# deno750/TSP_Optimization

Measured on AMD Instinct MI355X. Metric: 2opt_edge_pair_evals_per_sec, higher is better.
Workload: dtype f64

## Files before the change

tsp_optimization_amd/csrc/tsp_internal.hpp:

```cpp
#pragma once
#include <hip/hip_runtime.h>
#include <time.h>

#include <cstdint>
#include <cstdio>
#include <cstdlib>
#include <cstring>
#include <type_traits>
#include <vector>

#include "../../include/tsp_hip.h"
#include "tsp_dist.hpp"
#include "exh_arith.hpp"
#include "exh_decide.hpp"

namespace tsp {

struct alignas(16) Partial {
    double delta;
    int i, j;
};
static_assert(sizeof(Partial) == 16, "Partial must be 16 bytes");

struct alignas(16) TourState {
    int ci, cj;
    int chunk_rows;
    int done;
    double obj;
    double seen_cost;
    long long sweeps, evals, moves, reversed, pairs_scanned, steps;
    int parity, pending, mv_pa, mv_pb;
    long long lane_pairs, tier1_pairs, exact_pairs, staged_recs;
    int hit_rows;
    int open;
    int pad1, pad2;
};

constexpr int kScanThreads = 256;
constexpr int kApplyThreads = 1024;

}

#define TSP_SWITCH_LIST(X)                                                                                                  \
    X(ENGINE) X(CLUSTER_BLOCKS) X(CLUSTER_MIN_ROWS) X(CLUSTER_MAX_ROWS) X(CLUSTER_HIT_CAP) X(CLUSTER_SPIN_LIMIT)            \
    X(CLUSTER_SPIN_MS) X(CLUSTER_COPIES) X(CLUSTER_TILE_ROWS) X(CLUSTER_XCD_LOCAL) X(CLUSTER_ALLOW_OVERSUB) X(CLUSTER_DEBUG) X(CLUSTER_PROBE) X(CLUSTER_FIRST_SORTED) X(TABU_DENSE)     \
    X(LDS_PROBE) X(LDS_MIN_ROWS) X(LDS_EDGE_CACHE) X(NO_ICOORD) X(NO_FILTER) X(NO_PRUNE) X(SORTED_MIN_N)      \
    X(SWEEP_BLOCKS) X(SWEEP_TABLE) X(BEST_ROWS_PER_BLOCK) X(BEST_RECS) X(FIRST_GRID_ROWS) X(FIRST_MIN_ROWS)                \
    X(FIRST_MAX_ROWS) X(CONSTRUCT_GLOBAL) X(CONSTRUCT_NN) X(CLUSTER_FS_ROWS) X(LDS_F32_MIN_N) X(EXH_POS) X(TABU_INKERNEL) X(OROPT_FULL)
namespace tsp {
enum SwitchId {
#define TSP_SW_ENUM(name) SW_##name,
    TSP_SWITCH_LIST(TSP_SW_ENUM)
#undef TSP_SW_ENUM
    SW_COUNT
};
struct Switches {
    int v[SW_COUNT];
    bool has[SW_COUNT];
    int get(SwitchId k, int dflt) const { return has[k] ? v[k] : dflt; }
};
void read_switches(Switches *sw);
}
#define TSP_SW(inst_, NAME, dflt) ((inst_)->sw.get(tsp::SW_##NAME, (dflt)))


struct tsp_dev_ctx {
    int device = 0;
    hipStream_t stream = nullptr;
// ... 80 lines not shown
    bool exh_hot = false;
    int exh_share[4] = {0, 0, 0, 0};
    int exh_gens = 0;
    tsp::ExhDeal *d_exh_deal = nullptr;
    tsp::ExhCand *d_exh_cand = nullptr;
    int exh_lds = 0;
    int exh_blocks = 0;
    int *d_pairtab = nullptr;
    int *d_ticket = nullptr;
    int *d_row_ticket = nullptr;
    tsp::Partial *d_row_slot = nullptr;
    int *d_row_evals = nullptr;
    int max_tile_rows = 0;
    int *d_slot_evals = nullptr;
    unsigned long long *d_cl_slots = nullptr;
    size_t cl_slot_words = 0;
    int cl_C = 0;
    long long *d_cl_stats = nullptr;
    unsigned cl_epoch = 0;
    int *d_cl_pairtab = nullptr;
    int cl_ntests = 0;
    int *d_order_snap = nullptr;
    std::vector<double> h_obj_snap;
    int *d_kick_result = nullptr;
    int *h_kick_result = nullptr;
    int *d_chain = nullptr, *h_chain = nullptr;
    bool h_state_fresh = false;
    int *h_cl_err = nullptr;
    bool tabu_list_run = false;
    int *d_order0 = nullptr;
    std::vector<double> h_obj0;
    std::vector<int> h_order_buf;
    tsp::TourState *h_state = nullptr;
    int first_grid_rows = 32;
    int first_max_rows2 = 2048;
    int first_min_rows = 8;
    int best_rows_per_block = 32;
    int use_recs = 1;
    double device_ms = 0.0;
};

namespace tsp {
void set_last_error(const char *what, hipError_t e, const char *file, int line);
void set_last_error_text(const char *text);

template <typename T>
struct DevBuf {
    T *p = nullptr;
    DevBuf() = default;
    DevBuf(const DevBuf &) = delete;
    DevBuf &operator=(const DevBuf &) = delete;
    ~DevBuf() { if (p) (void)hipFree(p); }
    hipError_t alloc(size_t count) { return hipMalloc(&p, sizeof(T) * count); }
    operator T *() const { return p; }
};
}
namespace tsp {
struct HkTree {
    const int *d_elo = nullptr, *d_ehi = nullptr;
    const double *d_ew = nullptr, *d_pi = nullptr;
    double W = 0.0;
    long long rounds = 0;
    float device_ms = 0.f;
};
struct TabuRide {
    tsp_dev_tabu *tabu = nullptr;
// ... 73 lines not shown
```

tsp_optimization_amd/csrc/two_opt_exh.hpp:

```cpp
#pragma once
#include "two_opt_step.hpp"
#include "exh_arith.hpp"
#include "exh_decide.hpp"

#pragma clang fp contract(off)

namespace tsp {

#ifdef TSP_STAMPS
__device__ unsigned long long g_exh_w[8192 * 4];
__device__ unsigned long long g_exh_t[8];
__device__ unsigned long long g_exh_f[8192];
#endif

constexpr int kExhPad = 1152;
constexpr int kRowBatch = 4;
constexpr int kExhRJ = 4;

template <int WT>
constexpr bool exh_metric() { return WT == WT_EUC_2D_ICOORD || WT == WT_CEIL_2D_ICOORD || WT == WT_ATT_ICOORD; }

template <int WT>
constexpr int exh_mode() { return WT == WT_EUC_2D_ICOORD ? EXH_NINT : (WT == WT_CEIL_2D_ICOORD ? EXH_CEIL : EXH_ATT); }

// ... 89 lines not shown
    __syncthreads();
    d = s_d[0]; key = s_k[0];
    for (int w = 1; w < kScanThreads / 64; ++w)
        if (better(s_d[w], s_k[w], d, key)) { d = s_d[w]; key = s_k[w]; }
    if (key == kNoKey || !(d < 0)) return {0, -1, -1};
    const int delta = (int)d;
    bool ambiguous = false;
    for (int w = 0; w < kScanThreads / 64; ++w)
        ambiguous = ambiguous || (s_k[w] != kNoKey && s_d[w] == d && (s_amb[w] != 0 || s_k[w] != key));
    if (ambiguous) {
        ExhIdBest ib;
#pragma unroll
        for (int k = 0; k < kExhCandPU; ++k) exh_fold_ids(ib, one.c[k], delta, id_at);
        if (two) {
#pragma unroll
            for (int k = 0; k < kExhCandPU; ++k) exh_fold_ids(ib, more.c[k], delta, id_at);
        }
        u64 idkey = ib.idkey;
        double unused = 0.0;
        block_argmin<false>(unused, idkey, s_d, s_k);
        if (ib.idkey == idkey) s_pair = ib.poskey;
        __syncthreads();
        key = s_pair;
    }
    return {1, exh_key_hi(key), exh_key_lo(key)};
}

__device__ __forceinline__ SweepDecision exh_decision(const ExhMove &m) {
    SweepDecision d;
    d.found = 1; d.pa = m.pa; d.pb = m.pb; d.L = m.L;
    return d;
}

template <int WT, bool INT, bool HOT>
__global__ __launch_bounds__(kScanThreads) void k_move_pos(const TourState *__restrict__ states, const ExhCand *__restrict__ cands,
                                                           const ExhRec *__restrict__ rec_old, int cand_per_tour, int n,
                                                           ExhRec *__restrict__ rec, TourState *__restrict__ states_next,
                                                           const double2 *__restrict__ coord, int *orders, int *poss, int *orders2,
                                                           int *poss2) {
    static_assert(exh_metric<WT>() && INT, "integer-coordinate metrics only (integer costs: the tour cost needs no staging)");
    __shared__ double s_d[kScanThreads / 64];
    __shared__ u64 s_k[kScanThreads / 64];
    const int tour = blockIdx.y;
    const TourState *st = states + tour;
    const bool writer = blockIdx.x == 0 && threadIdx.x == 0;
    const ExhCand *cand = cands + (size_t)tour * cand_per_tour;
    const ExhCandLoads first = exh_cand_load(cand, cand_per_tour, threadIdx.x);
    int done = st->done, is_open = st->open, parity = st->parity, pending = st->pending, mv_pa = st->mv_pa, mv_pb = st->mv_pb;
    __builtin_amdgcn_sched_barrier(0);
    const int args_null = (int)(coord == nullptr) | (int)(orders == nullptr) | (int)(poss == nullptr) | (int)(orders2 == nullptr) |
                          (int)(poss2 == nullptr) | (int)(states_next == nullptr) | (int)(rec_old == nullptr) | (int)(rec == nullptr);
    asm volatile("" : "+s"(done), "+s"(is_open), "+s"(parity), "+s"(pending), "+s"(mv_pa), "+s"(mv_pb) : "s"(n), "s"(args_null));
    exh_cand_pin(first);
    if (done) {
        if (writer) states_next[tour] = *st;
        return;
    }
    const size_t base = (size_t)tour * n, pbase = (size_t)tour * (n + kExhPad);
    MoveView mv = move_view(parity, pending, mv_pa, mv_pb, orders + base, poss + base, orders2 + base, poss2 + base, n);
    const ExhRec *__restrict__ old = rec_old + pbase;
    const bool open = is_open != 0;
    SweepDecision dec;
    ExhPair pr = {0, -1, -1};
    if (open) {
        pr = exh_decide(first, cand, cand_per_tour, [&](int p) { if constexpr (HOT) return old[p].id; else return mv.order[p]; }, s_d, s_k);
        if (!pr.found) {
            if (blockIdx.x != 0) return;
            const double cost = tour_cost_block<WT, INT>(coord, mv.order, mv.pos, n, s_d, nullptr);
            if (writer) {
                TourState z = *st;
                sweep_count(z, dec, n, cost);
                z.pending = 0;
                states_next[tour] = z;
            }
            return;
        }
    }
    const int k = blockIdx.x * kScanThreads + threadIdx.x;
    if (k >= n + kExhPad) return;
    int u;
    ExhRec r;
    if constexpr (HOT) {
        ExhMove m1 = {mv_pa, mv_pb, mv.pa1, mv.L}, m2 = m1;
        if (open) { m1 = exh_orient(pr.p, pr.q, n, true); m2 = exh_orient(pr.p, pr.q, n, false); }
        const ExhPerm pm1 = exh_perm(k, n, m1.pa1, m1.L), pm2 = exh_perm(k, n, m2.pa1, m2.L);
        const ExhRec ra1 = old[pm1.a], rb1 = old[pm1.b], ra2 = old[pm2.a], rb2 = old[pm2.b];
        const int wrap = old[n].eprev;
        int idp = 0, idq = 1;
        if (open) { idp = old[pr.p].id; idq = old[pr.q].id; }
        __builtin_amdgcn_sched_barrier(0);
        asm volatile("" : : "v"(ra1.m2x), "v"(ra1.m2y), "v"(ra1.nrm), "v"(ra1.eprev), "v"(rb1.m2x), "v"(rb1.m2y), "v"(rb1.nrm),
                     "v"(rb1.eprev), "v"(rb1.id), "v"(wrap));
        asm volatile("" : : "v"(ra2.m2x), "v"(ra2.m2y), "v"(ra2.nrm), "v"(ra2.eprev), "v"(rb2.m2x), "v"(rb2.m2y), "v"(rb2.nrm),
                     "v"(rb2.eprev), "v"(rb2.id), "v"(idp), "v"(idq));
        const bool p_first = idp < idq;
        const ExhMove m = p_first ? m1 : m2;
        r = exh_perm_rec<exh_mode<WT>()>(p_first ? pm1 : pm2, p_first ? ra1 : ra2, p_first ? rb1 : rb2, wrap,
                                         [](double v) { return __builtin_amdgcn_sqrt(v); });
        u = r.id;
        mv.L = m.L; mv.pa1 = m.pa1;
        if (open) dec = exh_decision(m);
    } else {
        if (open) {
            const ExhMove m = exh_orient(pr.p, pr.q, n, mv.order[pr.p] < mv.order[pr.q]);
            mv.L = m.L; mv.pa1 = m.pa1;
            dec = exh_decision(m);
        }
        u = k < n ? mv.node_at(k) : (k == n ? mv.node_at(0) : -1);
        const int v = k >= 1 && k <= n ? mv.node_at(k - 1) : -1;
        const double2 c0 = coord[0];
        double2 cu = make_double2(c0.x - 6.0e6, c0.y - 6.0e6);
        int len = 0;
        if (u >= 0) cu = coord[u];
        if (v >= 0) { const double2 cv = coord[v]; len = (int)dist_xy<WT, INT>(cv.x, cv.y, cu.x, cu.y); }
        exh_rec_xy(cu.x - c0.x, cu.y - c0.y, r);
        r.eprev = len;
        r.id = u;
    }
    if (mv.L > 0 && k < n) {
        int *o_new = (parity ? orders : orders2) + base, *p_new = (parity ? poss : poss2) + base;
        o_new[k] = u;
        p_new[u] = k;
    }
    rec[pbase + k] = r;
    if (writer) {
        TourState z = *st;
        if (open) sweep_count(z, dec, n, 0.0);
        if (mv.L > 0) z.parity ^= 1;
        z.pending = 0;
        states_next[tour] = z;
    }
}

template <int WT, bool INT>
__global__ __launch_bounds__(kScanThreads) void k_exh_close(const double2 *__restrict__ coord, const int *orders, const int *poss,
                                                            const int *orders2, const int *poss2, TourState *states,
                                                            const ExhCand *__restrict__ cands, int cand_per_tour, int n) {
    static_assert(exh_metric<WT>() && INT, "integer-coordinate metrics only");
    __shared__ double s_d[kScanThreads / 64];
    __shared__ u64 s_k[kScanThreads / 64];
    const int tour = blockIdx.x;
    TourState *st = states + tour;
    if (st->done || !st->open) return;
    const size_t base = (size_t)tour * n;
    const bool second = st->parity != 0;
    const int *order = (second ? orders2 : orders) + base, *pos = (second ? poss2 : poss) + base;
    const ExhCand *cand = cands + (size_t)tour * cand_per_tour;
    const ExhPair pr = exh_decide(exh_cand_load(cand, cand_per_tour, threadIdx.x), cand, cand_per_tour,
                                  [&](int p) { return order[p]; }, s_d, s_k);
    SweepDecision dec;
    double cost = 0.0;
    if (pr.found) dec = exh_decision(exh_orient(pr.p, pr.q, n, order[pr.p] < order[pr.q]));
    else cost = tour_cost_block<WT, INT>(coord, order, pos, n, s_d, nullptr);
    if (threadIdx.x == 0) {
        TourState z = *st;
        sweep_count(z, dec, n, cost);
        z.pending = dec.found;
        *st = z;
    }
}

template <int WT, bool INT, int RJ>
__global__ __launch_bounds__(kScanThreads, 1) void k_exh(const TourState *__restrict__ states, const ExhRec *__restrict__ rec_all, int n,
                                                      int cand_per_tour, const ExhDeal *__restrict__ deal,
                                                      ExhCand *__restrict__ cand_all, TourState *states_w) {
    static_assert(exh_metric<WT>(), "integer-coordinate metrics only");
    constexpr int W = 64 * RJ, WEFF = W - 1;
#ifdef TSP_STAMPS
    const unsigned long long stamp_r0 = __builtin_amdgcn_s_memrealtime(), stamp_c0 = __builtin_amdgcn_s_memtime();
    unsigned long long stamp_hits = 0, stamp_hit_cycles = 0, stamp_first = 0;
#endif
    const int tour = blockIdx.z;
    const int tid = threadIdx.x, lane = tid & 63;
    const int gw = __builtin_amdgcn_readfirstlane((int)blockIdx.x * (kScanThreads / 64) + (tid >> 6));
    int done = states[tour].done;
    ExhDeal dl = deal[gw];
#ifdef TSP_STAMPS
    done = __builtin_amdgcn_readfirstlane(done);
    dl.strip = __builtin_amdgcn_readfirstlane(dl.strip); dl.row = __builtin_amdgcn_readfirstlane(dl.row);
    dl.count = (long long)(((u64)(unsigned)__builtin_amdgcn_readfirstlane((int)((u64)dl.count >> 32)) << 32) |
                           (unsigned)__builtin_amdgcn_readfirstlane((int)(u64)dl.count));
#endif
    const int args_null = (int)(rec_all == nullptr);
    asm volatile("" : "+s"(done), "+s"(dl.strip), "+s"(dl.row), "+s"(dl.count)
                 : "s"(n), "s"(args_null), "s"(cand_per_tour), "s"(cand_all), "s"(states_w));
    if (done) return;
// ... 154 lines not shown
```

tsp_optimization_amd/csrc/two_opt_grid.hip:

```cpp
#include "cluster_deal.hpp"
#include "tabu_chain.hpp"
#include "two_opt_exh.hpp"
#include "two_opt_first.hpp"
#include "two_opt_step.hpp"
#include "two_opt_sweep.hpp"
#include "two_opt_tiled.hpp"

#include <algorithm>

#pragma clang fp contract(off)
namespace tsp {

__global__ void k_stamp_scatter(int *__restrict__ stamp, const int *__restrict__ idx, const int *__restrict__ val,
                                int count) {
    const int t = blockIdx.x * blockDim.x + threadIdx.x;
    if (t < count) stamp[idx[t]] = val[t];
}
__global__ void k_stamp_gather(const int *__restrict__ stamp, const int *__restrict__ idx, int *__restrict__ val,
                               int count) {
    const int t = blockIdx.x * blockDim.x + threadIdx.x;
    if (t < count) val[t] = stamp[idx[t]];
}


// ... 171 lines not shown
}

int exh_cands(const tsp_dev_tours *t) { return t->exh_blocks; }

constexpr long long kTabuListMax = 16384;
constexpr long long kTabuCompactSlack = 256;

int tabu_list_prepare(tsp_dev_tours *t, tsp_dev_tabu *tb, bool *usable, long long room = 0 ) {
    *usable = false;
    if (t->B != 1 || !tb->d_list || t->n < 4) return TSP_OK;
    hipStream_t s = t->inst->ctx->stream;
    bool readback = false;
    if (!tb->list_valid) {
        TSP_HIP_TRY(hipMemsetAsync(tb->d_list_n, 0, sizeof(int), s));
        hipLaunchKernelGGL(k_tabu_scan, dim3(2048), dim3(256), 0, s, tb->d_stamp, tb->count, t->n, tb->d_list, tb->list_cap, tb->d_list_n);
        readback = true;
    } else if (tb->list_ub + room > tb->list_compact_at) {
        hipLaunchKernelGGL(k_tabu_compact, dim3(1), dim3(1024), 0, s, tb->d_stamp, t->n, tb->d_list, tb->d_list_n);
        readback = true;
    }
    if (readback) {
        TSP_HIP_TRY(hipMemcpyAsync(tb->h_list_n, tb->d_list_n, sizeof(int), hipMemcpyDeviceToHost, s));
        TSP_HIP_TRY(hipStreamSynchronize(s));
        TSP_HIP_TRY(hipGetLastError());
        const long long m = *tb->h_list_n;
        tb->list_valid = m <= tb->list_cap;
        tb->list_ub = m;
        tb->list_compact_at = m + std::max(kTabuCompactSlack, room);
    }
    *usable = tb->list_valid && tb->list_ub <= kTabuListMax;
    return TSP_OK;
}

struct ExhHotScope {
    tsp_dev_tours *t;
    explicit ExhHotScope(tsp_dev_tours *t_) : t(t_) { t->exh_hot = false; }
    ~ExhHotScope() { t->exh_hot = false; }
    ExhHotScope(const ExhHotScope &) = delete;
    ExhHotScope &operator=(const ExhHotScope &) = delete;
};

void launch_flush(tsp_dev_tours *t) {
    t->exh_hot = false;
    if (!t->d_order2) return;
    hipStream_t s = t->inst->ctx->stream;
    const dim3 g((t->n + 255) / 256, t->B);
    hipLaunchKernelGGL(k_flush_move, g, dim3(256), 0, s, t->d_order, t->d_pos, t->d_order2, t->d_pos2, t->d_state, t->n);
    hipLaunchKernelGGL(k_flush_copy, g, dim3(256), 0, s, t->d_order, t->d_pos, t->d_order2, t->d_pos2, t->d_state, t->n);
    hipLaunchKernelGGL(k_flush_state, dim3((t->B + 255) / 256), dim3(256), 0, s, t->d_state, t->B);
}

int exh_fill_deal(tsp_dev_tours *t) {
    const int waves_total = t->exh_blocks * (kScanThreads / 64);
    std::vector<ExhDeal> tab((size_t)waves_total);
    for (int gw = 0; gw < waves_total; ++gw) tab[(size_t)gw] = exh_deal(t->n, 64 * kExhRJ - 1, waves_total, t->exh_share, t->exh_gens, gw);
    if (!t->d_exh_deal) TSP_HIP_TRY(hipMalloc(&t->d_exh_deal, tab.size() * sizeof(ExhDeal)));
    TSP_HIP_TRY(hipMemcpy(t->d_exh_deal, tab.data(), tab.size() * sizeof(ExhDeal), hipMemcpyHostToDevice));
    return TSP_OK;
}

void launch_exh_close(tsp_dev_tours *t) {
    hipStream_t s = t->inst->ctx->stream;
    TSP_DISPATCH_METRIC(t->inst->wtype, t->inst->integer_cost, {
        if constexpr (exh_metric<WTC>())
            hipLaunchKernelGGL((k_exh_close<WTC, INTC>), dim3(t->B), dim3(kScanThreads), 0, s, t->inst->d_coord, t->d_order, t->d_pos,
                               t->d_order2, t->d_pos2, t->d_state, (const ExhCand *)t->d_exh_cand, exh_cands(t), t->n);
    });
}

StepArgs make_args(tsp_dev_tours *t, int mode, tsp_dev_tabu *tabu, int iter, int tenure) {
    StepArgs a;
    a.coord = t->inst->d_coord; a.orders = t->d_order; a.poss = t->d_pos; a.states = t->d_state;
    a.partials = t->d_partial; a.tickets = t->d_ticket; a.slot_evals = t->d_slot_evals;
    a.row_tickets = t->d_row_ticket; a.row_slots = t->d_row_slot; a.row_evals = t->d_row_evals;
    a.max_tile_rows = t->max_tile_rows;
    a.tabu = tabu ? tabu->d_stamp : nullptr;
    a.recs = (mode == TSP_2OPT_BEST && t->use_recs && t->n >= 4096) ? t->d_rec : nullptr;
    a.partial_per_tour = t->partial_per_tour;
    a.n = t->n;
    a.rows_per_block = t->best_rows_per_block;
    a.first_min_rows = std::min(t->first_min_rows, std::max(1, t->n - 1));
    a.first_max_rows = 0;
    a.iter = iter; a.tenure = tenure;
    a.margin = t->inst->filter_margin;
    a.prune = t->inst->prune_margin;
    a.sum_margin = t->inst->sum_margin;
    a.pairtab = t->d_pairtab;
    a.cl_tickets = t->d_cl_ticket;
    a.orders2 = t->d_order2; a.poss2 = t->d_pos2;
    a.gbox = t->inst->d_gbox; a.gmax = t->d_gmax;
    a.ng = t->inst->ng; a.n_slots = t->inst->n_slots;
    a.flat_slots = t->sweep_blocks;
    a.tabu_list = tabu ? tabu->d_list : nullptr; a.tabu_list_n = tabu ? tabu->d_list_n : nullptr;
    a.tabu_list_cap = tabu ? tabu->list_cap : 0; a.tabu_pairs = tabu ? tabu->d_tabu_pairs : nullptr;
    return a;
}

template <int WT, bool INT>
int launch_step(tsp_dev_tours *t, int mode, tsp_dev_tabu *tabu, int iter, int tenure) {
    hipStream_t s = t->inst->ctx->stream;
    StepArgs a = make_args(t, mode, tabu, iter, tenure);
    if constexpr (exh_metric<WT>()) {
        if (exh_run(t, mode, tabu)) {
            TourState *cur = t->d_state;
            t->slot ^= 1;
            t->d_state = t->d_state_base + (size_t)t->slot * t->B;
            const ExhRec *rec_old = t->exh_hot ? t->d_prec[t->exh_buf] : nullptr;
            t->exh_buf ^= 1;
            ExhRec *rec_new = t->d_prec[t->exh_buf];
            const dim3 gm((t->n + kExhPad + kScanThreads - 1) / kScanThreads, t->B);
            const ExhCand *cands = t->d_exh_cand;
            if (rec_old)
                hipLaunchKernelGGL((k_move_pos<WT, INT, true>), gm, dim3(kScanThreads), 0, s, cur, cands, rec_old, exh_cands(t), t->n,
                                   rec_new, t->d_state, t->inst->d_coord, t->d_order, t->d_pos, t->d_order2, t->d_pos2);
            else
                hipLaunchKernelGGL((k_move_pos<WT, INT, false>), gm, dim3(kScanThreads), 0, s, cur, cands, rec_old, exh_cands(t), t->n,
                                   rec_new, t->d_state, t->inst->d_coord, t->d_order, t->d_pos, t->d_order2, t->d_pos2);
            t->exh_hot = true;
            const dim3 g(t->exh_blocks, 1, t->B);
            hipLaunchKernelGGL((k_exh<WT, INT, kExhRJ>), g, dim3(kScanThreads), (size_t)t->exh_lds, s, (const TourState *)t->d_state,
                               (const ExhRec *)rec_new, t->n, exh_cands(t), (const ExhDeal *)t->d_exh_deal, t->d_exh_cand, t->d_state);
            return TSP_OK;
        }
    }
    if constexpr (has_root_filter<WT>()) {
        if (sorted_run(t, mode, tabu)) {
            a.recs = t->d_rec;
            const int ns = t->inst->n_slots;
            hipLaunchKernelGGL((k_move_recs<WT, INT>), dim3((std::max(ns, t->n) + kScanThreads - 1) / kScanThreads, t->B),
                               dim3(kScanThreads), 0, s, t->inst->d_coord, t->d_order, t->d_pos, t->d_order2, t->d_pos2,
                               t->d_state, t->inst->d_sperm, t->d_rec, t->d_gmax, t->n, t->inst->ng, ns);
            if (tabu)
                hipLaunchKernelGGL((k_sweep<WT, INT, true>), dim3(t->sweep_blocks + kTabuSideBlocks, 1, t->B), dim3(kScanThreads), 0, s, a);
            else
                hipLaunchKernelGGL((k_sweep<WT, INT>), dim3(t->sweep_blocks, 1, t->B), dim3(kScanThreads), 0, s, a);
            return TSP_OK;
        }
    }
    if (mode == TSP_2OPT_BEST) {
        const dim3 g = best_grid(t);
        if (a.recs)
            hipLaunchKernelGGL((k_recs<WT, INT>), dim3((t->n + kScanThreads - 1) / kScanThreads, t->B), dim3(kScanThreads), 0, s,
                               t->inst->d_coord, t->d_order, t->d_pos, t->d_state, t->d_rec, t->n);
        if (tabu && t->tabu_list_run) {
            hipLaunchKernelGGL(k_tabu_side, dim3(kTabuSideBlocks), dim3(kScanThreads), 0, s, t->d_order, t->d_pos, t->n, t->d_state,
                               tabu->d_stamp, tabu->d_list, tabu->d_list_n, tabu->list_cap, iter, tenure, tabu->d_tabu_pairs);
            hipLaunchKernelGGL((k_step<WT, INT, TSP_2OPT_BEST, kBestRJ, false, true>), g, dim3(kScanThreads), 0, s, a);
        } else if (tabu)
            hipLaunchKernelGGL((k_step<WT, INT, TSP_2OPT_BEST, kBestRJ, true>), g, dim3(kScanThreads), 0, s, a);
        else
// ... 32 lines not shown
    hipStream_t s = t->inst->ctx->stream;
    TSP_DISPATCH_METRIC(t->inst->wtype, t->inst->integer_cost, {
        hipLaunchKernelGGL((k_tour_cost<WTC, INTC>), dim3(t->B), dim3(kApplyThreads), 0, s, t->inst->d_coord,
                           t->d_order, t->d_pos, t->n, d_out, stride_bytes);
    });
}


}

int tsp_grid_tour_cost(tsp_dev_tours *t, double *d_out) {
    launch_tour_cost(t, d_out, sizeof(double));
    TSP_HIP_TRY(hipGetLastError());
    return TSP_OK;
}

int tsp_grid_run(tsp_dev_tours *t, int mode, tsp_dev_tabu *tabu, int iter, int tenure, int64_t max_steps,
                 double time_limit_s, int sync, int *all_done) {
    if (!t || (mode != TSP_2OPT_FIRST && mode != TSP_2OPT_BEST)) return TSP_DEV_E_ARG;
    if (!sync && max_steps < 0) return TSP_DEV_E_ARG;
    ExhHotScope exh_hot_scope(t);
    hipStream_t s = t->inst->ctx->stream;
    const double t0 = wall_s();
    if (tabu && (iter < 0 || tenure < 0)) tabu = nullptr;
    t->tabu_list_run = false;
    if (tabu && mode == TSP_2OPT_BEST) {
        bool usable = false;
        const int rc = tabu_list_prepare(t, tabu, &usable);
        if (rc) return rc;
        t->tabu_list_run = usable && TSP_SW(t->inst, TABU_DENSE, 0) == 0;
        tabu->last_run_list = t->tabu_list_run;
        if (t->tabu_list_run) TSP_HIP_TRY(hipMemsetAsync(tabu->d_tabu_pairs, 0, kTabuSideWords * sizeof(unsigned long long), s));
    }
    const int64_t batch = 64;
    int64_t burst = sync ? 8 : batch;
    int64_t queued = 0;
    int status = TSP_OK;
    bool finished = false;
    if (all_done) *all_done = 0;
    const bool exh = exh_run(t, mode, tabu);
    if (!exh) launch_arm(t, mode);
    for (;;) {
        int64_t todo = burst;
        burst = std::min(batch, burst * 2);
        if (max_steps >= 0) todo = std::min<int64_t>(todo, max_steps - queued);
        if (todo <= 0) break;
        for (int64_t k = 0; k < todo; ++k) {
            int rc = launch_step_rt(t, mode, tabu, iter, tenure);
            if (rc) {
                if (exh) { launch_exh_close(t); launch_flush(t); }
                return rc;
            }
        }
        queued += todo;
        TSP_HIP_TRY(hipGetLastError());
        if (!sync) continue;
        if (exh) launch_exh_close(t);
        TSP_HIP_TRY(hipMemcpyAsync(t->h_state, t->d_state, sizeof(TourState) * (size_t)t->B, hipMemcpyDeviceToHost, s));
        TSP_HIP_TRY(hipStreamSynchronize(s));
        bool done = true;
        for (int b = 0; b < t->B; ++b) done = done && t->h_state[b].done;
        if (done) { finished = true; if (all_done) *all_done = 1; break; }
        if (time_limit_s > 0 && wall_s() - t0 > time_limit_s) { status = TSP_TIME_LIMIT_EXCEEDED; break; }
    }
    if (tabu && t->tabu_list_run)
        hipLaunchKernelGGL(k_tabu_fix_evals, dim3(1), dim3(64), 0, s, t->d_state, tabu->d_tabu_pairs);
    if (exh && !sync) launch_exh_close(t);
    if (sorted_run(t, mode, tabu) || exh || mode == TSP_2OPT_FIRST) {
        launch_flush(t);
        TSP_HIP_TRY(hipGetLastError());
        if (sync == 1) TSP_HIP_TRY(hipStreamSynchronize(s));
    }
    if ((status == TSP_TIME_LIMIT_EXCEEDED || (sync && !finished)) && mode == TSP_2OPT_BEST) {
        launch_tour_cost(t, &t->d_state[0].obj, sizeof(TourState));
        TSP_HIP_TRY(hipStreamSynchronize(s));
    }
    return status;
}

int tsp_grid_after_external_run(tsp_dev_tours *t, int mode, int timed_out, bool pos_written) {
    hipStream_t s = t->inst->ctx->stream;
    if (!pos_written) hipLaunchKernelGGL(k_build_pos, dim3((t->n + 255) / 256, t->B), dim3(256), 0, s, t->d_order, t->d_pos, t->n);
    if (timed_out && mode == TSP_2OPT_BEST) {
        launch_tour_cost(t, &t->d_state[0].obj, sizeof(TourState));
        TSP_HIP_TRY(hipStreamSynchronize(s));
    }
    TSP_HIP_TRY(hipGetLastError());
    return TSP_OK;
}

void tsp_grid_tabu_follow(tsp_dev_tours *t, const TabuRide &r, int k, const int *d_err) {
    hipStream_t s = t->inst->ctx->stream;
    tsp_dev_tabu *tabu = r.tabu;
    if (r.follow == TabuRide::kPost) {
        hipLaunchKernelGGL(k_tabu_post, dim3(1), dim3(kApplyThreads), 0, s, t->d_state, d_err, t->d_order, t->d_pos, tabu->d_stamp, t->n,
                           r.a, r.b, r.iter, r.tenure, t->d_kick_result, tabu->list_valid ? tabu->d_list : nullptr, tabu->d_list_n,
// ... 332 lines not shown
    t->sorted_min_n = TSP_SW(inst, SORTED_MIN_N, 1000);
    t->cl_sorted_min_n = TSP_SW(inst, SORTED_MIN_N, 8);
    size_t rec_per_tour = (size_t)inst->n;
    size_t cl_words = (size_t)B * 64 * 64;
    if (inst->d_sperm) {
        const long long gp = (long long)inst->ng * (inst->ng + 1) / 2;
        const int one_tour = (int)std::min<long long>(768, std::max<long long>(256, gp / 8));
        const int want = TSP_SW(inst, SWEEP_BLOCKS, std::max(16, one_tour / B));
        t->sweep_blocks = std::max(1, want / kSweepCluster) * kSweepCluster;
        rec_per_tour = std::max(rec_per_tour, (size_t)inst->n_slots);
        t->partial_per_tour = std::max(t->partial_per_tour, (size_t)t->sweep_blocks);
        cl_words = std::max(cl_words, (size_t)B * (t->sweep_blocks / kSweepCluster) * 64);
        const long long npairs = (long long)inst->ng * (inst->ng + 1) / 2;
        if (npairs <= (1ll << 24) && inst->ng <= 32768 && TSP_SW(inst, SWEEP_TABLE, 1)) {
            std::vector<int> tab;
            cluster_deal(reinterpret_cast<const double *>(inst->h_gbox.data()), nullptr, nullptr, nullptr, inst->n, inst->ng,
                         t->sweep_blocks / kSweepCluster, false, 1.0, tab);
            TSP_HIP_TRY(hipMalloc(&t->d_pairtab, tab.size() * sizeof(int)));
            TSP_HIP_TRY(hipMemcpy(t->d_pairtab, tab.data(), tab.size() * sizeof(int), hipMemcpyHostToDevice));
        }
        TSP_HIP_TRY(hipMalloc(&t->d_gmax, (size_t)B * (inst->ng + 1) * sizeof(double)));

    }
    if (inst->filter_margin > 1e299 && TSP_SW(inst, EXH_POS, 1) && inst->n >= 5 &&
        (inst->wtype == WT_EUC_2D_ICOORD || inst->wtype == WT_CEIL_2D_ICOORD || inst->wtype == WT_ATT_ICOORD)) {
        constexpr int waves = 4;
        t->exh_blocks = std::max(1, std::min(2048, inst->ctx->num_cus * waves / std::max(1, B > 4 ? 4 : B)));
        if (B == 1 && inst->ctx->lds_bytes >= 65536)
            t->exh_lds = std::min(65536, inst->ctx->lds_bytes / waves) - 1024;
        static_assert(2048 <= kExhMaxCand, "exh_decide takes a tour's candidates in two rounds at the most");
        const size_t pn = (size_t)B * (inst->n + kExhPad);
        TSP_HIP_TRY(hipMalloc(&t->d_prec[0], pn * sizeof(ExhRec)));
        TSP_HIP_TRY(hipMalloc(&t->d_prec[1], pn * sizeof(ExhRec)));
        TSP_HIP_TRY(hipMalloc(&t->d_exh_cand, (size_t)B * exh_cands(t) * sizeof(ExhCand)));
        TSP_HIP_TRY(hipMemset(t->d_exh_cand, 0xff, (size_t)B * exh_cands(t) * sizeof(ExhCand)));
        {
            t->exh_share[0] = t->exh_share[1] = t->exh_share[2] = t->exh_share[3] = 0;
            t->exh_gens = 0;
            int pc[4] = {45, 29, 16, 10};
            bool on = B == 1;
            const char *e = getenv("TSP_EXH_SHARES");
            if (e && *e) {
                pc[0] = pc[1] = pc[2] = pc[3] = 0;
                const int got = sscanf(e, "%d,%d,%d,%d", &pc[0], &pc[1], &pc[2], &pc[3]);
                on = on && got == waves && pc[0] > 0;
            }
            const long long total = exh_total_rows(inst->n, 64 * kExhRJ - 1);
            const long long wtot = (long long)t->exh_blocks * (kScanThreads / 64);
            const int sum = pc[0] + pc[1] + pc[2] + pc[3];
            if (on && sum > 0 && wtot % waves == 0) {
                const long long wq = wtot / waves;
                t->exh_gens = waves;
                for (int q = 0; q < waves; ++q) t->exh_share[q] = (int)std::max<long long>(1, (total * pc[q] + sum * wq - 1) / (sum * wq));
            }
            const int rc = exh_fill_deal(t);
            if (rc) return rc;
        }
    }
    TSP_HIP_TRY(hipMalloc(&t->d_cl_ticket, cl_words * sizeof(int)));
    TSP_HIP_TRY(hipMemset(t->d_cl_ticket, 0, cl_words * sizeof(int)));
    TSP_HIP_TRY(hipMalloc(&t->d_order, bn * sizeof(int)));
    TSP_HIP_TRY(hipMalloc(&t->d_order2, bn * sizeof(int)));
    TSP_HIP_TRY(hipMalloc(&t->d_pos2, bn * sizeof(int)));
    TSP_HIP_TRY(hipMalloc(&t->d_order0, bn * sizeof(int)));
    TSP_HIP_TRY(hipMalloc(&t->d_pos, bn * sizeof(int)));
    TSP_HIP_TRY(hipMalloc(&t->d_state_base, 2 * (size_t)B * sizeof(TourState)));
    t->d_state = t->d_state_base; t->slot = 0;
    TSP_HIP_TRY(hipMalloc(&t->d_partial, (size_t)B * t->partial_per_tour * sizeof(Partial)));
    TSP_HIP_TRY(hipMalloc(&t->d_slot_evals, (size_t)B * t->partial_per_tour * sizeof(int)));
    TSP_HIP_TRY(hipMalloc(&t->d_ticket, (size_t)B * sizeof(int)));
    t->use_recs = TSP_SW(inst, BEST_RECS, 1);
    TSP_HIP_TRY(hipMalloc(&t->d_rec, (size_t)B * rec_per_tour * sizeof(NodeRec)));
    t->max_tile_rows = (int)gb.y;
    TSP_HIP_TRY(hipMalloc(&t->d_row_ticket, (size_t)B * t->max_tile_rows * sizeof(int)));
    TSP_HIP_TRY(hipMalloc(&t->d_row_evals, (size_t)B * t->max_tile_rows * sizeof(int)));
    TSP_HIP_TRY(hipMalloc(&t->d_row_slot, (size_t)B * t->max_tile_rows * sizeof(Partial)));
    TSP_HIP_TRY(hipHostMalloc(&t->h_state, (size_t)B * sizeof(TourState)));
    guard.t = nullptr;
    *out = t;
    return TSP_OK;
}

void tsp_dev_tours_destroy(tsp_dev_tours *t) {
    if (!t) return;
    (void)hipSetDevice(t->inst->ctx->device);
    (void)hipStreamSynchronize(t->inst->ctx->stream);
    (void)hipFree(t->d_order); (void)hipFree(t->d_order0); (void)hipFree(t->d_pos);
    (void)hipFree(t->d_state_base); (void)hipFree(t->d_partial); (void)hipFree(t->d_slot_evals); (void)hipFree(t->d_ticket); (void)hipFree(t->d_rec);
    (void)hipFree(t->d_gmax); (void)hipFree(t->d_order2); (void)hipFree(t->d_pos2); (void)hipFree(t->d_pairtab); (void)hipFree(t->d_cl_ticket);
    (void)hipFree(t->d_row_ticket); (void)hipFree(t->d_row_evals); (void)hipFree(t->d_row_slot);
    (void)hipFree(t->d_prec[0]); (void)hipFree(t->d_prec[1]); (void)hipFree(t->d_exh_deal); (void)hipFree(t->d_exh_cand);
    (void)hipFree(t->d_cl_slots); (void)hipFree(t->d_cl_pairtab); (void)hipFree(t->d_cl_stats);
    (void)hipFree(t->d_chain); (void)hipHostFree(t->h_chain); (void)hipFree(t->d_order_snap); (void)hipFree(t->d_kick_result); (void)hipHostFree(t->h_kick_result); (void)hipHostFree(t->h_cl_err);
    (void)hipHostFree(t->h_state);
    delete t;
}

int tsp_dev_tours_reset(tsp_dev_tours *t) {
    if (!t) return TSP_DEV_E_ARG;
    hipStream_t s = t->inst->ctx->stream;
    const int n = t->n, B = t->B;
    TSP_HIP_TRY(hipMemcpyAsync(t->d_order, t->d_order0, (size_t)B * n * sizeof(int), hipMemcpyDeviceToDevice, s));
    hipLaunchKernelGGL(k_build_pos, dim3((n + 255) / 256, B), dim3(256), 0, s, t->d_order, t->d_pos, n);
    for (int b = 0; b < B; ++b) {
        TourState z;
        memset(&z, 0, sizeof z);
        z.chunk_rows = std::min(t->first_min_rows, std::max(1, n - 1));
        z.obj = t->h_obj0[b];
        z.seen_cost = t->h_obj0[b];
        t->h_state[b] = z;
    }
    t->slot = 0; t->d_state = t->d_state_base;
    if (t->d_cl_stats) TSP_HIP_TRY(hipMemsetAsync(t->d_cl_stats, 0, sizeof(long long) * (size_t)B * 256 * 4, s));
    TSP_HIP_TRY(hipMemcpyAsync(t->d_state, t->h_state, sizeof(TourState) * (size_t)B, hipMemcpyHostToDevice, s));
    TSP_HIP_TRY(hipStreamSynchronize(s));
    TSP_HIP_TRY(hipGetLastError());
    return TSP_OK;
}

int tsp_dev_tours_upload(tsp_dev_tours *t, const int *succ, int succ_stride, int64_t tour_stride, const double *obj) {
    if (!t || !succ || succ_stride < 1) return TSP_DEV_E_ARG;
    const int n = t->n, B = t->B;
    hipStream_t s = t->inst->ctx->stream;
    std::vector<int> &order = t->h_order_buf;
    order.resize((size_t)B * n);
    std::vector<char> seen((size_t)n);
    for (int b = 0; b < B; ++b) {
// ... 315 lines not shown
```

tsp_optimization_amd/csrc/two_opt_sweep.hpp:

```cpp
#pragma once
#include "two_opt_step.hpp"
#include "two_opt_tabu_list.hpp"

#pragma clang fp contract(off)

namespace tsp {

template <int WT, bool INT>
__global__ __launch_bounds__(kScanThreads) void k_move_recs(const double2 *__restrict__ coord, int *orders, int *poss,
                                                            int *orders2, int *poss2, const TourState *__restrict__ states,
                                                            const int *__restrict__ sperm, NodeRec *__restrict__ recs,
                                                            double *__restrict__ gmax, int n, int ng, int n_slots) {
    const int tour = blockIdx.y;
    const TourState *st = states + tour;
    if (st->done) return;
    const size_t base = (size_t)tour * n;
    const MoveView mv = move_view(st, orders + base, poss + base, orders2 + base, poss2 + base, n);
    const int k = blockIdx.x * kScanThreads + threadIdx.x;
    const bool copies = mv.L > 0 && k < n;
    const int moved = copies ? mv.node_at(k) : 0;
    const int v = k < n_slots ? sperm[k] : -1;
    NodeRec r;
    if (v >= 0) {
        int ps = mv.pos_of(v) + 1; if (ps == n) ps = 0;
// ... 12 lines not shown
    }
    if (k >= n_slots) return;
    recs[(size_t)tour * n_slots + k] = r;
    const u64 mb = ~wave_min_u64(~(u64)__double_as_longlong(r.ds));
    if ((threadIdx.x & 63) == 0) gmax[(size_t)tour * (ng + 1) + (k >> 6)] = __longlong_as_double((long long)mb);
}

__global__ void k_flush_move(int *orders, int *poss, int *orders2, int *poss2, const TourState *__restrict__ states, int n) {
    const int tour = blockIdx.y;
    const TourState *st = states + tour;
    if (!st->pending) return;
    const size_t base = (size_t)tour * n;
    const MoveView mv = move_view(st, orders + base, poss + base, orders2 + base, poss2 + base, n);
    const int k = blockIdx.x * blockDim.x + threadIdx.x;
    if (k >= n) return;
    int *o_new = (st->parity ? orders : orders2) + base, *p_new = (st->parity ? poss : poss2) + base;
    const int v = mv.node_at(k);
    o_new[k] = v;
    p_new[v] = k;
}
__global__ void k_flush_copy(int *orders, int *poss, const int *orders2, const int *poss2,
                             const TourState *__restrict__ states, int n) {
    const int tour = blockIdx.y;
    const TourState *st = states + tour;
    if ((st->parity ^ st->pending) == 0) return;
    const int k = blockIdx.x * blockDim.x + threadIdx.x;
    if (k >= n) return;
    const size_t base = (size_t)tour * n;
    orders[base + k] = orders2[base + k];
    poss[base + k] = poss2[base + k];
}
__global__ void k_flush_state(TourState *states, int B) {
    const int b = blockIdx.x * blockDim.x + threadIdx.x;
    if (b < B) { states[b].parity = 0; states[b].pending = 0; }
}

__device__ __forceinline__ double lane_bcast(double v, int l) {
    const int lo = __builtin_amdgcn_readlane(__double2loint(v), l), hi = __builtin_amdgcn_readlane(__double2hiint(v), l);
    return __hiloint2double(hi, lo);
}

__device__ __forceinline__ void group_pair(int t, int ng, int &r, int &c) {
    const double b = 2.0 * ng + 1.0;
    int rr = (int)((b - sqrt(b * b - 8.0 * (double)t)) * 0.5);
    rr = max(0, min(rr, ng - 1));
    while (rr > 0 && (long long)rr * ng - (long long)rr * (rr - 1) / 2 > t) --rr;
    while ((long long)(rr + 1) * ng - (long long)(rr + 1) * rr / 2 <= t) ++rr;
    r = rr;
    c = rr + (int)(t - ((long long)rr * ng - (long long)rr * (rr - 1) / 2));
}

constexpr int kSweepCluster = 4;
constexpr int kSweepRows = 16;
constexpr int kSweepStage = 8;
constexpr int kSweepListCap = 1024;

template <int WT, bool INT, bool TABU = false>
__global__ __launch_bounds__(kScanThreads, 3) void k_sweep(const StepArgs a) {
    constexpr bool ATT10 = WT == WT_ATT || WT == WT_ATT_ICOORD;
    constexpr int NW = kScanThreads / 64;
#ifdef TSP_STAMPS
    __shared__ unsigned long long stamps[16];
#endif
    TSP_STAMP(0);
    const int tour = blockIdx.z;
    const TourState *st = a.states + tour;
    if (st->done) return;
// ... 219 lines not shown
```

Before: 1588 billion.

## Keep hot exhaustive 2-opt tour in records and pipeline host state polling

In the hot exhaustive path, the move kernel no longer writes order/pos arrays and only touches the n+1 live record slots. Pad records are initialized once at allocation, and a settle kernel rebuilds order/pos from the record buffer only at flush. Tour cost and the close decision are now read from record edge lengths instead of recomputed from coordinates. The synchronous loop double-buffers the state readback with events so the host checks the previous batch while the next one runs, at the cost of extra in-flight batches and more state bookkeeping.

```diff
diff --git a/tsp_optimization_amd/csrc/tsp_internal.hpp b/tsp_optimization_amd/csrc/tsp_internal.hpp
--- a/tsp_optimization_amd/csrc/tsp_internal.hpp
+++ b/tsp_optimization_amd/csrc/tsp_internal.hpp
@@ -33,7 +33,8 @@
     long long lane_pairs, tier1_pairs, exact_pairs, staged_recs;
     int hit_rows;
     int open;
-    int pad1, pad2;
+    int rec_buf;
+    int pad2;
 };
 
 constexpr int kScanThreads = 256;
@@ -180,6 +181,7 @@
     std::vector<double> h_obj0;
     std::vector<int> h_order_buf;
     tsp::TourState *h_state = nullptr;
+    hipEvent_t poll_ev[2] = {nullptr, nullptr};
     int first_grid_rows = 32;
     int first_max_rows2 = 2048;
     int first_min_rows = 8;
diff --git a/tsp_optimization_amd/csrc/two_opt_exh.hpp b/tsp_optimization_amd/csrc/two_opt_exh.hpp
--- a/tsp_optimization_amd/csrc/two_opt_exh.hpp
+++ b/tsp_optimization_amd/csrc/two_opt_exh.hpp
@@ -145,12 +145,45 @@
     return d;
 }
 
+__device__ __forceinline__ double exh_rec_cost(const ExhRec *__restrict__ rec, int n, double *s_d) {
+    double c = 0.0;
+    for (int k = 1 + (int)threadIdx.x; k <= n; k += (int)blockDim.x) c += (double)rec[k].eprev;
+    return block_sum<double>(c, s_d);
+}
+
+__global__ void k_exh_pads(const double2 *__restrict__ coord, ExhRec *__restrict__ rec_a, ExhRec *__restrict__ rec_b, int n) {
+    const int k = n + 1 + blockIdx.x * blockDim.x + threadIdx.x;
+    if (k >= n + kExhPad) return;
+    const double2 c0 = coord[0];
+    const double2 cu = make_double2(c0.x - 6.0e6, c0.y - 6.0e6);
+    ExhRec r;
+    exh_rec_xy(cu.x - c0.x, cu.y - c0.y, r);
+    r.eprev = 0;
+    r.id = -1;
+    const size_t at = (size_t)blockIdx.y * (n + kExhPad) + k;
+    rec_a[at] = r;
+    rec_b[at] = r;
+}
+
+__global__ void k_exh_settle(const ExhRec *__restrict__ rec_a, const ExhRec *__restrict__ rec_b, const TourState *__restrict__ states,
+                             int *orders, int *poss, int *orders2, int *poss2, int n) {
+    const int tour = blockIdx.y, k = blockIdx.x * blockDim.x + threadIdx.x;
+    const int mark = states[tour].rec_buf;
+    if (k >= n || mark == 0) return;
+    const bool second = states[tour].parity != 0;
+    const size_t base = (size_t)tour * n;
+    const int u = (mark == 1 ? rec_a : rec_b)[(size_t)tour * (n + kExhPad) + k].id;
+    if ((unsigned)u >= (unsigned)n) return;
+    ((second ? orders2 : orders) + base)[k] = u;
+    ((second ? poss2 : poss) + base)[u] = k;
+}
+
 template <int WT, bool INT, bool HOT>
 __global__ __launch_bounds__(kScanThreads) void k_move_pos(const TourState *__restrict__ states, const ExhCand *__restrict__ cands,
                                                            const ExhRec *__restrict__ rec_old, int cand_per_tour, int n,
                                                            ExhRec *__restrict__ rec, TourState *__restrict__ states_next,
                                                            const double2 *__restrict__ coord, int *orders, int *poss, int *orders2,
-                                                           int *poss2) {
+                                                           int *poss2, int rec_mark) {
     static_assert(exh_metric<WT>() && INT, "integer-coordinate metrics only (integer costs: the tour cost needs no staging)");
     __shared__ double s_d[kScanThreads / 64];
     __shared__ u64 s_k[kScanThreads / 64];
@@ -179,7 +212,9 @@
         pr = exh_decide(first, cand, cand_per_tour, [&](int p) { if constexpr (HOT) return old[p].id; else return mv.order[p]; }, s_d, s_k);
         if (!pr.found) {
             if (blockIdx.x != 0) return;
-            const double cost = tour_cost_block<WT, INT>(coord, mv.order, mv.pos, n, s_d, nullptr);
+            double cost;
+            if constexpr (HOT) cost = exh_rec_cost(old, n, s_d);
+            else cost = tour_cost_block<WT, INT>(coord, mv.order, mv.pos, n, s_d, nullptr);
             if (writer) {
                 TourState z = *st;
                 sweep_count(z, dec, n, cost);
@@ -190,7 +225,7 @@
         }
     }
     const int k = blockIdx.x * kScanThreads + threadIdx.x;
-    if (k >= n + kExhPad) return;
+    if (k >= (HOT ? n + 1 : n + kExhPad)) return;
     int u;
     ExhRec r;
     if constexpr (HOT) {
@@ -230,24 +265,26 @@
         r.eprev = len;
         r.id = u;
     }
-    if (mv.L > 0 && k < n) {
-        int *o_new = (parity ? orders : orders2) + base, *p_new = (parity ? poss : poss2) + base;
-        o_new[k] = u;
-        p_new[u] = k;
+    if constexpr (!HOT) {
+        if (mv.L > 0 && k < n) {
+            int *o_new = (parity ? orders : orders2) + base, *p_new = (parity ? poss : poss2) + base;
+            o_new[k] = u;
+            p_new[u] = k;
+        }
     }
     rec[pbase + k] = r;
     if (writer) {
         TourState z = *st;
         if (open) sweep_count(z, dec, n, 0.0);
-        if (mv.L > 0) z.parity ^= 1;
+        if (!HOT && mv.L > 0) z.parity ^= 1;
         z.pending = 0;
+        z.rec_buf = rec_mark;
         states_next[tour] = z;
     }
 }
 
 template <int WT, bool INT>
-__global__ __launch_bounds__(kScanThreads) void k_exh_close(const double2 *__restrict__ coord, const int *orders, const int *poss,
-                                                            const int *orders2, const int *poss2, TourState *states,
+__global__ __launch_bounds__(kScanThreads) void k_exh_close(const ExhRec *__restrict__ rec_all, TourState *states,
                                                             const ExhCand *__restrict__ cands, int cand_per_tour, int n) {
     static_assert(exh_metric<WT>() && INT, "integer-coordinate metrics only");
     __shared__ double s_d[kScanThreads / 64];
@@ -255,16 +292,14 @@
     const int tour = blockIdx.x;
     TourState *st = states + tour;
     if (st->done || !st->open) return;
-    const size_t base = (size_t)tour * n;
-    const bool second = st->parity != 0;
-    const int *order = (second ? orders2 : orders) + base, *pos = (second ? poss2 : poss) + base;
+    const ExhRec *__restrict__ rec = rec_all + (size_t)tour * (n + kExhPad);
     const ExhCand *cand = cands + (size_t)tour * cand_per_tour;
     const ExhPair pr = exh_decide(exh_cand_load(cand, cand_per_tour, threadIdx.x), cand, cand_per_tour,
-                                  [&](int p) { return order[p]; }, s_d, s_k);
+                                  [&](int p) { return rec[p].id; }, s_d, s_k);
     SweepDecision dec;
     double cost = 0.0;
-    if (pr.found) dec = exh_decision(exh_orient(pr.p, pr.q, n, order[pr.p] < order[pr.q]));
-    else cost = tour_cost_block<WT, INT>(coord, order, pos, n, s_d, nullptr);
+    if (pr.found) dec = exh_decision(exh_orient(pr.p, pr.q, n, rec[pr.p].id < rec[pr.q].id));
+    else cost = exh_rec_cost(rec, n, s_d);
     if (threadIdx.x == 0) {
         TourState z = *st;
         sweep_count(z, dec, n, cost);
diff --git a/tsp_optimization_amd/csrc/two_opt_grid.hip b/tsp_optimization_amd/csrc/two_opt_grid.hip
--- a/tsp_optimization_amd/csrc/two_opt_grid.hip
+++ b/tsp_optimization_amd/csrc/two_opt_grid.hip
@@ -227,19 +227,24 @@
     return TSP_OK;
 }
 
+void launch_flush(tsp_dev_tours *t);
+
 struct ExhHotScope {
     tsp_dev_tours *t;
     explicit ExhHotScope(tsp_dev_tours *t_) : t(t_) { t->exh_hot = false; }
-    ~ExhHotScope() { t->exh_hot = false; }
+    ~ExhHotScope() { if (t->exh_hot) launch_flush(t); }
     ExhHotScope(const ExhHotScope &) = delete;
     ExhHotScope &operator=(const ExhHotScope &) = delete;
 };
 
 void launch_flush(tsp_dev_tours *t) {
+    hipStream_t s = t->inst->ctx->stream;
+    const dim3 g((t->n + 255) / 256, t->B);
+    if (t->exh_hot)
+        hipLaunchKernelGGL(k_exh_settle, g, dim3(256), 0, s, (const ExhRec *)t->d_prec[0], (const ExhRec *)t->d_prec[1],
+                           (const TourState *)t->d_state, t->d_order, t->d_pos, t->d_order2, t->d_pos2, t->n);
     t->exh_hot = false;
     if (!t->d_order2) return;
-    hipStream_t s = t->inst->ctx->stream;
-    const dim3 g((t->n + 255) / 256, t->B);
     hipLaunchKernelGGL(k_flush_move, g, dim3(256), 0, s, t->d_order, t->d_pos, t->d_order2, t->d_pos2, t->d_state, t->n);
     hipLaunchKernelGGL(k_flush_copy, g, dim3(256), 0, s, t->d_order, t->d_pos, t->d_order2, t->d_pos2, t->d_state, t->n);
     hipLaunchKernelGGL(k_flush_state, dim3((t->B + 255) / 256), dim3(256), 0, s, t->d_state, t->B);
@@ -258,8 +263,8 @@
     hipStream_t s = t->inst->ctx->stream;
     TSP_DISPATCH_METRIC(t->inst->wtype, t->inst->integer_cost, {
         if constexpr (exh_metric<WTC>())
-            hipLaunchKernelGGL((k_exh_close<WTC, INTC>), dim3(t->B), dim3(kScanThreads), 0, s, t->inst->d_coord, t->d_order, t->d_pos,
-                               t->d_order2, t->d_pos2, t->d_state, (const ExhCand *)t->d_exh_cand, exh_cands(t), t->n);
+            hipLaunchKernelGGL((k_exh_close<WTC, INTC>), dim3(t->B), dim3(kScanThreads), 0, s, (const ExhRec *)t->d_prec[t->exh_buf],
+                               t->d_state, (const ExhCand *)t->d_exh_cand, exh_cands(t), t->n);
     });
 }
 
@@ -303,14 +308,15 @@
             const ExhRec *rec_old = t->exh_hot ? t->d_prec[t->exh_buf] : nullptr;
             t->exh_buf ^= 1;
             ExhRec *rec_new = t->d_prec[t->exh_buf];
-            const dim3 gm((t->n + kExhPad + kScanThreads - 1) / kScanThreads, t->B);
+            const dim3 gm((t->n + kExhPad + kScanThreads - 1) / kScanThreads, t->B), gh((t->n + 1 + kScanThreads - 1) / kScanThreads, t->B);
             const ExhCand *cands = t->d_exh_cand;
+            const int mark = t->exh_buf + 1;
             if (rec_old)
-                hipLaunchKernelGGL((k_move_pos<WT, INT, true>), gm, dim3(kScanThreads), 0, s, cur, cands, rec_old, exh_cands(t), t->n,
-                                   rec_new, t->d_state, t->inst->d_coord, t->d_order, t->d_pos, t->d_order2, t->d_pos2);
+                hipLaunchKernelGGL((k_move_pos<WT, INT, true>), gh, dim3(kScanThreads), 0, s, cur, cands, rec_old, exh_cands(t), t->n,
+                                   rec_new, t->d_state, t->inst->d_coord, t->d_order, t->d_pos, t->d_order2, t->d_pos2, mark);
             else
                 hipLaunchKernelGGL((k_move_pos<WT, INT, false>), gm, dim3(kScanThreads), 0, s, cur, cands, rec_old, exh_cands(t), t->n,
-                                   rec_new, t->d_state, t->inst->d_coord, t->d_order, t->d_pos, t->d_order2, t->d_pos2);
+                                   rec_new, t->d_state, t->inst->d_coord, t->d_order, t->d_pos, t->d_order2, t->d_pos2, mark);
             t->exh_hot = true;
             const dim3 g(t->exh_blocks, 1, t->B);
             hipLaunchKernelGGL((k_exh<WT, INT, kExhRJ>), g, dim3(kScanThreads), (size_t)t->exh_lds, s, (const TourState *)t->d_state,
@@ -409,14 +415,23 @@
         tabu->last_run_list = t->tabu_list_run;
         if (t->tabu_list_run) TSP_HIP_TRY(hipMemsetAsync(tabu->d_tabu_pairs, 0, kTabuSideWords * sizeof(unsigned long long), s));
     }
-    const int64_t batch = 64;
+    const bool exh = exh_run(t, mode, tabu);
+    const bool piped = exh && sync && !(time_limit_s > 0);
+    const int64_t batch = piped ? 32 : 64;
     int64_t burst = sync ? 8 : batch;
     int64_t queued = 0;
     int status = TSP_OK;
     bool finished = false;
     if (all_done) *all_done = 0;
-    const bool exh = exh_run(t, mode, tabu);
     if (!exh) launch_arm(t, mode);
+    int64_t polls = 0;
+    auto look = [&](int64_t k, bool *done) -> int {
+        TSP_HIP_TRY(hipEventSynchronize(t->poll_ev[k & 1]));
+        memcpy(t->h_state, t->h_state + (size_t)(1 + (k & 1)) * t->B, sizeof(TourState) * (size_t)t->B);
+        *done = true;
+        for (int b = 0; b < t->B; ++b) *done = *done && t->h_state[b].done;
+        return TSP_OK;
+    };
     for (;;) {
         int64_t todo = burst;
         burst = std::min(batch, burst * 2);
@@ -432,13 +447,31 @@
         queued += todo;
         TSP_HIP_TRY(hipGetLastError());
         if (!sync) continue;
-        if (exh) launch_exh_close(t);
+        if (exh && (!piped || (max_steps >= 0 && queued >= max_steps))) launch_exh_close(t);
+        if (piped) {
+            TSP_HIP_TRY(hipMemcpyAsync(t->h_state + (size_t)(1 + (polls & 1)) * t->B, t->d_state, sizeof(TourState) * (size_t)t->B,
+                                       hipMemcpyDeviceToHost, s));
+            TSP_HIP_TRY(hipEventRecord(t->poll_ev[polls & 1], s));
+            ++polls;
+            if (polls < 2) continue;
+            bool done = false;
+            const int rc = look(polls - 2, &done);
+            if (rc) return rc;
+            if (done) { finished = true; if (all_done) *all_done = 1; break; }
+            continue;
+        }
         TSP_HIP_TRY(hipMemcpyAsync(t->h_state, t->d_state, sizeof(TourState) * (size_t)t->B, hipMemcpyDeviceToHost, s));
         TSP_HIP_TRY(hipStreamSynchronize(s));
         bool done = true;
         for (int b = 0; b < t->B; ++b) done = done && t->h_state[b].done;
         if (done) { finished = true; if (all_done) *all_done = 1; break; }
         if (time_limit_s > 0 && wall_s() - t0 > time_limit_s) { status = TSP_TIME_LIMIT_EXCEEDED; break; }
+    }
+    if (piped && !finished && polls > 0) {
+        bool done = false;
+        const int rc = look(polls - 1, &done);
+        if (rc) return rc;
+        if (done) { finished = true; if (all_done) *all_done = 1; }
     }
     if (tabu && t->tabu_list_run)
         hipLaunchKernelGGL(k_tabu_fix_evals, dim3(1), dim3(64), 0, s, t->d_state, tabu->d_tabu_pairs);
@@ -837,6 +870,9 @@
         const size_t pn = (size_t)B * (inst->n + kExhPad);
         TSP_HIP_TRY(hipMalloc(&t->d_prec[0], pn * sizeof(ExhRec)));
         TSP_HIP_TRY(hipMalloc(&t->d_prec[1], pn * sizeof(ExhRec)));
+        hipLaunchKernelGGL(k_exh_pads, dim3((kExhPad - 1 + 255) / 256, B), dim3(256), 0, inst->ctx->stream,
+                           (const double2 *)inst->d_coord, t->d_prec[0], t->d_prec[1], inst->n);
+        TSP_HIP_TRY(hipGetLastError());
         TSP_HIP_TRY(hipMalloc(&t->d_exh_cand, (size_t)B * exh_cands(t) * sizeof(ExhCand)));
         TSP_HIP_TRY(hipMemset(t->d_exh_cand, 0xff, (size_t)B * exh_cands(t) * sizeof(ExhCand)));
         {
@@ -880,7 +916,8 @@
     TSP_HIP_TRY(hipMalloc(&t->d_row_ticket, (size_t)B * t->max_tile_rows * sizeof(int)));
     TSP_HIP_TRY(hipMalloc(&t->d_row_evals, (size_t)B * t->max_tile_rows * sizeof(int)));
     TSP_HIP_TRY(hipMalloc(&t->d_row_slot, (size_t)B * t->max_tile_rows * sizeof(Partial)));
-    TSP_HIP_TRY(hipHostMalloc(&t->h_state, (size_t)B * sizeof(TourState)));
+    TSP_HIP_TRY(hipHostMalloc(&t->h_state, 3 * (size_t)B * sizeof(TourState)));
+    for (hipEvent_t &e : t->poll_ev) TSP_HIP_TRY(hipEventCreateWithFlags(&e, hipEventDisableTiming));
     guard.t = nullptr;
     *out = t;
     return TSP_OK;
@@ -898,6 +935,7 @@
     (void)hipFree(t->d_cl_slots); (void)hipFree(t->d_cl_pairtab); (void)hipFree(t->d_cl_stats);
     (void)hipFree(t->d_chain); (void)hipHostFree(t->h_chain); (void)hipFree(t->d_order_snap); (void)hipFree(t->d_kick_result); (void)hipHostFree(t->h_kick_result); (void)hipHostFree(t->h_cl_err);
     (void)hipHostFree(t->h_state);
+    for (hipEvent_t e : t->poll_ev) if (e) (void)hipEventDestroy(e);
     delete t;
 }
 
diff --git a/tsp_optimization_amd/csrc/two_opt_sweep.hpp b/tsp_optimization_amd/csrc/two_opt_sweep.hpp
--- a/tsp_optimization_amd/csrc/two_opt_sweep.hpp
+++ b/tsp_optimization_amd/csrc/two_opt_sweep.hpp
@@ -68,7 +68,7 @@
 }
 __global__ void k_flush_state(TourState *states, int B) {
     const int b = blockIdx.x * blockDim.x + threadIdx.x;
-    if (b < B) { states[b].parity = 0; states[b].pending = 0; }
+    if (b < B) { states[b].parity = 0; states[b].pending = 0; states[b].rec_buf = 0; }
 }
 
 __device__ __forceinline__ double lane_bcast(double v, int l) {
```

After: 1614 billion, median of 6. 1.02x the previous value.
